# MoonLab-YH/AOD_MEH_HUA

Hardware: AMD Instinct MI355X
Metric: images/sec train+HUA-score, RetinaNet-R50 VOC 512^2 (higher is better)
Workload: dtype bf16x3

## Files before the change

### aod_meh_hua_amd/csrc/bottleneck_x3.hip

```cpp
#include "common.h"

namespace {

struct Bnx3Args {
  const bf16_t* x;
  const bf16_t* w1;
  const bf16_t* w2;
  const bf16_t* w3;
  const float* s1; const float* b1; const float* s2; const float* b2; const float* s3; const float* b3;
  const bf16_t* res;
  const bf16_t* wd; const float* sd; const float* bd;
  bf16_t* y;
  int B, H, W, CP, tiles_y, tiles_x;
  int st3;
};

constexpr int TH = 8, TW = 16, HW_ = 18, HPIX = (TH + 2) * HW_;
constexpr int M1 = 192;
constexpr int XBUF = M1 * 128;
constexpr int OFF_W1 = 2 * XBUF;
constexpr int OFF_T1 = 65536;
constexpr int T1SUB = M1 * 128, T2SUB = TH * TW * 128;
constexpr int OFF_VEC = OFF_T1 + 2 * T1SUB;
constexpr int NVEC = 1280;
constexpr int OFF_WD = OFF_VEC + NVEC * 4;
constexpr int LDS_BYTES = OFF_WD, LDS_BYTES_DS = OFF_WD + 32768;
constexpr int SLOT = 8192;
constexpr int W3SUB = 256 * 128;
static_assert(OFF_W1 + 2 * 8192 <= OFF_T1 && 8 * SLOT <= OFF_T1 && 2 * W3SUB <= OFF_T1 && 2 * T2SUB <= 2 * T1SUB && LDS_BYTES_DS <= 160 * 1024, "LDS map");

template <int N> __device__ __forceinline__ void wait_vm() { asm volatile("s_waitcnt vmcnt(%0)" ::"n"(N) : "memory"); }
#ifdef AOD_TILE_TIMING
__device__ unsigned long long* g_b64_stamps = nullptr;
#define BSTAMP(k) do { if (g_b64_stamps && threadIdx.x == 0) g_b64_stamps[(size_t)blockIdx.x * 8 + (k)] = wall_clock64(); } while (0)
#else
#define BSTAMP(k) do {} while (0)
#endif

__device__ __forceinline__ int xcd_remap(int bid, int nwg) {
  const int q = nwg >> 3, r = nwg & 7, xcd = bid & 7, j = bid >> 3;
  return (xcd < r ? xcd * (q + 1) : r * (q + 1) + (xcd - r) * q) + j;
}
__device__ __forceinline__ int swz(int row, int chunk) { return row * 128 + ((chunk ^ ((row >> 1) & 7)) << 4); }
__device__ __forceinline__ int wswz(int row, int chunk) { return row * 128 + ((chunk ^ ((row >> 1) & 7) ^ (((row >> 4) & 1) << 1)) << 4); }
__device__ __forceinline__ int wrow(int j, int lr) { return (j >> 1) * 32 + (lr >> 2) * 8 + (j & 1) * 4 + (lr & 3); }

__device__ __forceinline__ void split8(const float (&v)[8], bf16x8& h, bf16x8& l) {
#pragma unroll
  for (int j = 0; j < 8; ++j) { h[j] = (bf16_t)v[j]; l[j] = (bf16_t)(v[j] - (float)h[j]); }
}

template <bool DS>
__global__ __launch_bounds__(512) __attribute__((amdgpu_waves_per_eu(2, 2))) void bottleneck64x3_fwd_kernel(const Bnx3Args p) {
  extern __shared__ __attribute__((aligned(16))) char smem[];
  typedef unsigned u32x4_t __attribute__((ext_vector_type(4)));
  const int t = threadIdx.x, lane = t & 63;
  BSTAMP(0);
  const int uw = __builtin_amdgcn_readfirstlane(t >> 6);
  const int lr = lane & 15, lq = lane >> 4;
  const int ntile = p.tiles_y * p.tiles_x;
  const int wg = xcd_remap(blockIdx.x, p.B * ntile);
  const int b = wg / ntile, tt = wg - b * ntile;
  const int ty0 = (tt / p.tiles_x) * TH, tx0 = (tt % p.tiles_x) * TW;
  const long long img0 = (long long)b * p.H * p.W;
  const long long npix = (long long)p.B * p.H * p.W;
  const auto rsrc_x = __builtin_amdgcn_make_buffer_rsrc((void*)p.x, 0, (int)(npix * p.CP * 2), 0x00020000);
  const auto rsrc_w1 = __builtin_amdgcn_make_buffer_rsrc((void*)p.w1, 0, 64 * p.CP * 2, 0x00020000);
  const auto rsrc_w2 = __builtin_amdgcn_make_buffer_rsrc((void*)p.w2, 0, 64 * 9 * 128 * 2, 0x00020000);
  const auto rsrc_w3 = __builtin_amdgcn_make_buffer_rsrc((void*)p.w3, 0, 256 * 128 * 2, 0x00020000);
  const auto rsrc_res = __builtin_amdgcn_make_buffer_rsrc((void*)(DS ? p.x : p.res), 0, DS ? (int)(npix * p.CP * 2) : (int)(npix * 1024), 0x00020000);
  const auto rsrc_wd = __builtin_amdgcn_make_buffer_rsrc((void*)p.wd, 0, DS ? 256 * 128 * 2 : 0, 0x00020000);
  const auto rsrc_y = __builtin_amdgcn_make_buffer_rsrc((void*)p.y, 0, (int)(npix * 1024), 0x00020000);
  constexpr unsigned OOB = 0xf0000000u;
  const int drow = lane >> 3;
  const int kc = (lane & 7) ^ ((4 * (uw & 1) + (lane >> 4)) & 7);
  const int kcw = kc ^ (((uw >> 1) & 1) << 1);

  auto halo_pix = [&](int h, int& y, int& x) -> bool {
    const int hy = h / HW_, hx = h - hy * HW_;
    y = ty0 - 1 + hy; x = tx0 - 1 + hx;
    return h < HPIX && (unsigned)y < (unsigned)p.H && (unsigned)x < (unsigned)p.W;
  };
  float* const vec = reinterpret_cast<float*>(smem + OFF_VEC);
  {
    float v;
    if (t < 64) v = p.s1[t];
    else if (t < 128) v = p.b1[t - 64];
    else if (t < 192) v = p.s2[t - 128];
    else if (t < 256) v = p.b2[t - 192];
    else v = p.s3[t - 256];
    vec[t] = v;
    if (t < 256) vec[512 + t] = p.b3[t];
    if constexpr (DS) {
      if (t < 256) vec[768 + t] = p.sd[t]; else vec[768 + t] = p.bd[t - 256];
    }
  }
  const float* const vs1 = vec, * const vb1 = vec + 64, * const vs2 = vec + 128, * const vb2 = vec + 192, * const vs3 = vec + 256, * const vb3 = vec + 512;
  const float* const vsd = vec + 768, * const vbd = vec + 1024;
  const unsigned wdlane = (unsigned)((8 * uw + drow) * 256 + kcw * 16);
  auto issueD = [&](int half) {
#pragma unroll
    for (int g = 0; g < 2; ++g)
#pragma unroll
      for (int i = 0; i < 2; ++i)
        __builtin_amdgcn_raw_ptr_buffer_load_lds(rsrc_wd, (__attribute__((address_space(3))) void*)(smem + OFF_WD + g * 16384 + (uw + 8 * i) * 1024), 16,
                                                 wdlane + (unsigned)((half * 128 + i * 64) * 256) + (unsigned)g * 128u, 0, 0, 0);
  };
  if constexpr (DS) issueD(0);

  unsigned xoff[3];
#pragma unroll
  for (int i = 0; i < 3; ++i) {
    const int h = 8 * (uw + 8 * i) + drow;
    int y, x;
    xoff[i] = halo_pix(h, y, x) ? (unsigned)(((img0 + (long long)y * p.W + x) * p.CP + kc * 8) * 2) : OOB;
  }
  unsigned w1off = (unsigned)(((8 * uw + drow) * p.CP + kcw * 8) * 2);
  const int nk1 = p.CP >> 6;
  auto xstage = [&](int buf) -> char* { return smem + (buf < 2 ? buf * XBUF : OFF_T1); };
  auto wstage = [&](int buf) -> char* { return smem + (buf < 2 ? OFF_W1 + buf * 8192 : OFF_T1 + XBUF); };
  static_assert(OFF_T1 + XBUF + 8192 <= OFF_VEC, "third phase-1 stage inside the t1 region");
  auto issue1 = [&](int buf) {
    char* xs = xstage(buf);
#pragma unroll
    for (int i = 0; i < 3; ++i) {
      const unsigned off = xoff[i];
      __builtin_amdgcn_raw_ptr_buffer_load_lds(rsrc_x, (__attribute__((address_space(3))) void*)(xs + (uw + 8 * i) * 1024), 16, off, 0, 0, 0);
      xoff[i] += 128;
    }
    __builtin_amdgcn_raw_ptr_buffer_load_lds(rsrc_w1, (__attribute__((address_space(3))) void*)(wstage(buf) + uw * 1024), 16, w1off, 0, 0, 0);
    w1off += 128;
  };
  const bool two = uw < 4;
  f32x4 acc1[2][4];
#pragma unroll
  for (int i = 0; i < 2; ++i)
#pragma unroll
    for (int j = 0; j < 4; ++j) acc1[i][j] = (f32x4){0.f, 0.f, 0.f, 0.f};
  const int nst = p.st3 ? 3 : 2;
  issue1(0);
  if (nk1 > 1) issue1(1);
  if (nst > 2 && nk1 > 2) issue1(2);
  int buf = 0;
  for (int kt = 0; kt < nk1; ++kt) {
    const int young = min(nk1 - 1 - kt, nst - 1);
    if (young >= 2) wait_vm<8>(); else if (young == 1) wait_vm<4>(); else wait_vm<0>();
    __builtin_amdgcn_s_barrier();
    __builtin_amdgcn_sched_barrier(0);
    const char* xs = xstage(buf);
    const char* ws = wstage(buf);
    bf16x8 wh[4], wl[4];
#pragma unroll
    for (int j = 0; j < 4; ++j) {
      wh[j] = *reinterpret_cast<const bf16x8*>(ws + wswz(wrow(j, lr), lq));
      wl[j] = *reinterpret_cast<const bf16x8*>(ws + wswz(wrow(j, lr), 4 + lq));
    }
#pragma unroll
    for (int i = 0; i < 2; ++i) {
      if (i == 0 || two) {
        const int row = (uw + 8 * i) * 16 + lr;
        const bf16x8 xh = *reinterpret_cast<const bf16x8*>(xs + swz(row, lq)), xl = *reinterpret_cast<const bf16x8*>(xs + swz(row, 4 + lq));
#pragma unroll
        for (int j = 0; j < 4; ++j) {
          acc1[i][j] = __builtin_amdgcn_mfma_f32_16x16x32_bf16(wh[j], xh, acc1[i][j], 0, 0, 0);
          acc1[i][j] = __builtin_amdgcn_mfma_f32_16x16x32_bf16(wh[j], xl, acc1[i][j], 0, 0, 0);
          acc1[i][j] = __builtin_amdgcn_mfma_f32_16x16x32_bf16(wl[j], xh, acc1[i][j], 0, 0, 0);
        }
      }
    }
    __builtin_amdgcn_sched_barrier(0);
    asm volatile("s_waitcnt lgkmcnt(0)" ::: "memory");
    __builtin_amdgcn_s_barrier();
    if (kt + nst < nk1) issue1(buf);
    buf = buf == nst - 1 ? 0 : buf + 1;
  }
  BSTAMP(1);
  const unsigned w2lane = (unsigned)(((8 * uw + drow) * (9 * 128) + kcw * 8) * 2);
  auto issue2 = [&](int s) {
    __builtin_amdgcn_raw_ptr_buffer_load_lds(rsrc_w2, (__attribute__((address_space(3))) void*)(smem + (s & 7) * SLOT + uw * 1024), 16,
                                             w2lane + (unsigned)s * 128u, 0, 0, 0);
  };
#pragma unroll
  for (int s = 0; s < 8; ++s) issue2(s);
  {
    char* t1 = smem + OFF_T1;
#pragma unroll
    for (int i = 0; i < 2; ++i) {
      if (i == 0 || two) {
        const int h = (uw + 8 * i) * 16 + lr;
        int y, x;
        const bool ok = halo_pix(h, y, x);
#pragma unroll
        for (int jp = 0; jp < 2; ++jp) {
          const int c = jp * 32 + lq * 8;
          float v[8];
#pragma unroll
          for (int q = 0; q < 2; ++q) {
            const f32x4 sc = *reinterpret_cast<const f32x4*>(vs1 + c + 4 * q), sh = *reinterpret_cast<const f32x4*>(vb1 + c + 4 * q);
#pragma unroll
            for (int r = 0; r < 4; ++r) v[4 * q + r] = ok ? fmaxf(acc1[i][2 * jp + q][r] * sc[r] + sh[r], 0.f) : 0.f;
          }
          bf16x8 oh, ol;
          split8(v, oh, ol);
          *reinterpret_cast<bf16x8*>(t1 + jp * T1SUB + swz(h, lq)) = oh;
          *reinterpret_cast<bf16x8*>(t1 + jp * T1SUB + swz(h, 4 + lq)) = ol;
        }
      }
    }
  }

  BSTAMP(2);
  f32x4 acc2[4];
#pragma unroll
  for (int j = 0; j < 4; ++j) acc2[j] = (f32x4){0.f, 0.f, 0.f, 0.f};
  const unsigned w3lane = (unsigned)((8 * uw + drow) * 256 + kcw * 16);
  auto issue3 = [&](int g) {
#pragma unroll
    for (int i = 0; i < 4; ++i)
      __builtin_amdgcn_raw_ptr_buffer_load_lds(rsrc_w3, (__attribute__((address_space(3))) void*)(smem + g * W3SUB + (uw + 8 * i) * 1024), 16,
                                               w3lane + (unsigned)(i * 64 * 256) + (unsigned)g * 128u, 0, 0, 0);
  };
#pragma unroll
  for (int G = 0; G < 5; ++G) {
    const int nst = G < 4 ? 4 : 2;
    if (G == 0) wait_vm<4>();
    else if (G == 1) wait_vm<4>();
    else if (G == 2) wait_vm<4>();
    else if (G == 3) wait_vm<2>();
    else wait_vm<4>();
    asm volatile("s_waitcnt lgkmcnt(0)" ::: "memory");
    __builtin_amdgcn_s_barrier();
    __builtin_amdgcn_sched_barrier(0);
#pragma unroll
    for (int k = 0; k < nst; ++k) {
      const int s = 4 * G + k, tap = s >> 1, g = s & 1;
      const int r = tap / 3, q = tap - r * 3;
      const char* ws = smem + (s & 7) * SLOT;
      const char* t1 = smem + OFF_T1 + g * T1SUB;
      const int row = (uw + r) * HW_ + lr + q;
      const bf16x8 ah = *reinterpret_cast<const bf16x8*>(t1 + swz(row, lq)), al = *reinterpret_cast<const bf16x8*>(t1 + swz(row, 4 + lq));
#pragma unroll
      for (int j = 0; j < 4; ++j) {
        const bf16x8 fh = *reinterpret_cast<const bf16x8*>(ws + wswz(wrow(j, lr), lq)), fl = *reinterpret_cast<const bf16x8*>(ws + wswz(wrow(j, lr), 4 + lq));
        acc2[j] = __builtin_amdgcn_mfma_f32_16x16x32_bf16(fh, ah, acc2[j], 0, 0, 0);
        acc2[j] = __builtin_amdgcn_mfma_f32_16x16x32_bf16(fh, al, acc2[j], 0, 0, 0);
        acc2[j] = __builtin_amdgcn_mfma_f32_16x16x32_bf16(fl, ah, acc2[j], 0, 0, 0);
      }
    }
    __builtin_amdgcn_sched_barrier(0);
    asm volatile("s_waitcnt lgkmcnt(0)" ::: "memory");
    __builtin_amdgcn_s_barrier();
    if (G < 3) {
#pragma unroll
      for (int k = 0; k < 4; ++k) if (4 * (G + 2) + k < 18) issue2(4 * (G + 2) + k);
    } else if (G == 3) issue3(1);
    else issue3(0);
  }
  BSTAMP(3);
  {
    char* t2 = smem + OFF_T1;
    const int o_ = uw * 16 + lr;
#pragma unroll
    for (int jp = 0; jp < 2; ++jp) {
      const int c = jp * 32 + lq * 8;
      float v[8];
#pragma unroll
      for (int q = 0; q < 2; ++q) {
        const f32x4 sc = *reinterpret_cast<const f32x4*>(vs2 + c + 4 * q), sh = *reinterpret_cast<const f32x4*>(vb2 + c + 4 * q);
#pragma unroll
        for (int r = 0; r < 4; ++r) v[4 * q + r] = fmaxf(acc2[2 * jp + q][r] * sc[r] + sh[r], 0.f);
      }
      bf16x8 oh, ol;
      split8(v, oh, ol);
      *reinterpret_cast<bf16x8*>(t2 + jp * T2SUB + swz(o_, lq)) = oh;
      *reinterpret_cast<bf16x8*>(t2 + jp * T2SUB + swz(o_, 4 + lq)) = ol;
    }
  }
  const int oy = ty0 + uw, ox = tx0 + lr;
  const unsigned prow = (oy < p.H && ox < p.W) ? (unsigned)((img0 + (long long)oy * p.W + ox) * 1024) : OOB;
  u32x4_t rh[4], rl[4];
  auto load_res = [&](int half) {
#pragma unroll
    for (int jp = 0; jp < 4; ++jp) {
      const int c = half * 128 + jp * 32 + lq * 8;
      const unsigned col = (unsigned)((((c >> 5) << 6) + (c & 31)) * 2);
      rh[jp] = __builtin_amdgcn_raw_buffer_load_b128(rsrc_res, (int)(prow + col), 0, 0);
      rl[jp] = __builtin_amdgcn_raw_buffer_load_b128(rsrc_res, (int)(prow + col + 64u), 0, 0);
    }
  };
  u32x4_t xf[4];
  auto load_xf = [&]() {
    const unsigned xrow = (oy < p.H && ox < p.W) ? (unsigned)((img0 + (long long)oy * p.W + ox) * 256) : OOB;
#pragma unroll
    for (int q = 0; q < 4; ++q) xf[q] = __builtin_amdgcn_raw_buffer_load_b128(rsrc_res, (int)(xrow + (unsigned)(q * 64 + lq * 16)), 0, 0);
  };
  auto compute_res = [&](int half) {
    f32x4 accd[8];
#pragma unroll
    for (int j = 0; j < 8; ++j) accd[j] = (f32x4){0.f, 0.f, 0.f, 0.f};
#pragma unroll
    for (int g = 0; g < 2; ++g) {
      const char* ws = smem + OFF_WD + g * 16384;
      const bf16x8 ah = __builtin_bit_cast(bf16x8, xf[2 * g]), al = __builtin_bit_cast(bf16x8, xf[2 * g + 1]);
#pragma unroll
      for (int j = 0; j < 8; ++j) {
        const int fr = wrow(j, lr);
        const bf16x8 fh = *reinterpret_cast<const bf16x8*>(ws + wswz(fr, lq)), fl = *reinterpret_cast<const bf16x8*>(ws + wswz(fr, 4 + lq));
        accd[j] = __builtin_amdgcn_mfma_f32_16x16x32_bf16(fh, ah, accd[j], 0, 0, 0);
        accd[j] = __builtin_amdgcn_mfma_f32_16x16x32_bf16(fh, al, accd[j], 0, 0, 0);
        accd[j] = __builtin_amdgcn_mfma_f32_16x16x32_bf16(fl, ah, accd[j], 0, 0, 0);
      }
    }
#pragma unroll
    for (int jp = 0; jp < 4; ++jp) {
      const int c = half * 128 + jp * 32 + lq * 8;
      float v[8];
#pragma unroll
      for (int h2 = 0; h2 < 2; ++h2) {
        const f32x4 sc = *reinterpret_cast<const f32x4*>(vsd + c + 4 * h2), sh = *reinterpret_cast<const f32x4*>(vbd + c + 4 * h2);
#pragma unroll
        for (int r = 0; r < 4; ++r) v[4 * h2 + r] = accd[2 * jp + h2][r] * sc[r] + sh[r];
      }
      bf16x8 oh, ol;
      split8(v, oh, ol);
      rh[jp] = __builtin_bit_cast(u32x4_t, oh); rl[jp] = __builtin_bit_cast(u32x4_t, ol);
    }
  };
  wait_vm<0>();
  if constexpr (DS) load_xf(); else load_res(0);
  asm volatile("s_waitcnt lgkmcnt(0)" ::: "memory");
  __builtin_amdgcn_s_barrier();
  __builtin_amdgcn_sched_barrier(0);
  BSTAMP(4);

#pragma unroll
  for (int half = 0; half < 2; ++half) {
    if constexpr (DS) {
      if (half == 1) {
        wait_vm<12>();
        __builtin_amdgcn_s_barrier();
        __builtin_amdgcn_sched_barrier(0);
      }
      compute_res(half);
      if (half == 0) {
        __builtin_amdgcn_sched_barrier(0);
        asm volatile("s_waitcnt lgkmcnt(0)" ::: "memory");
        __builtin_amdgcn_s_barrier();
        issueD(1);
        __builtin_amdgcn_sched_barrier(0);
      }
    }
    f32x4 acc3[8];
#pragma unroll
    for (int j = 0; j < 8; ++j) acc3[j] = (f32x4){0.f, 0.f, 0.f, 0.f};
#pragma unroll
    for (int g = 0; g < 2; ++g) {
      const char* t2 = smem + OFF_T1 + g * T2SUB;
      const char* ws = smem + g * W3SUB;
      const int row = uw * 16 + lr;
      const bf16x8 ah = *reinterpret_cast<const bf16x8*>(t2 + swz(row, lq)), al = *reinterpret_cast<const bf16x8*>(t2 + swz(row, 4 + lq));
#pragma unroll
      for (int j = 0; j < 8; ++j) {
        const int fr = half * 128 + wrow(j, lr);
        const bf16x8 fh = *reinterpret_cast<const bf16x8*>(ws + wswz(fr, lq)), fl = *reinterpret_cast<const bf16x8*>(ws + wswz(fr, 4 + lq));
        acc3[j] = __builtin_amdgcn_mfma_f32_16x16x32_bf16(fh, ah, acc3[j], 0, 0, 0);
        acc3[j] = __builtin_amdgcn_mfma_f32_16x16x32_bf16(fh, al, acc3[j], 0, 0, 0);
        acc3[j] = __builtin_amdgcn_mfma_f32_16x16x32_bf16(fl, ah, acc3[j], 0, 0, 0);
      }
    }
#pragma unroll
    for (int jp = 0; jp < 4; ++jp) {
      const int c = half * 128 + jp * 32 + lq * 8;
      const u32x4_t qh = rh[jp], ql = rl[jp];
      float v[8];
#pragma unroll
      for (int h2 = 0; h2 < 2; ++h2) {
        const f32x4 sc = *reinterpret_cast<const f32x4*>(vs3 + c + 4 * h2), sh = *reinterpret_cast<const f32x4*>(vb3 + c + 4 * h2);
#pragma unroll
        for (int r = 0; r < 4; ++r) v[4 * h2 + r] = acc3[2 * jp + h2][r] * sc[r] + sh[r];
        v[4 * h2 + 0] += __uint_as_float(qh[2 * h2] << 16) + __uint_as_float(ql[2 * h2] << 16);
        v[4 * h2 + 1] += __uint_as_float(qh[2 * h2] & 0xffff0000u) + __uint_as_float(ql[2 * h2] & 0xffff0000u);
        v[4 * h2 + 2] += __uint_as_float(qh[2 * h2 + 1] << 16) + __uint_as_float(ql[2 * h2 + 1] << 16);
        v[4 * h2 + 3] += __uint_as_float(qh[2 * h2 + 1] & 0xffff0000u) + __uint_as_float(ql[2 * h2 + 1] & 0xffff0000u);
      }
#pragma unroll
      for (int r = 0; r < 8; ++r) v[r] = fmaxf(v[r], 0.f);
      bf16x8 oh, ol;
      split8(v, oh, ol);
      const unsigned col = (unsigned)((((c >> 5) << 6) + (c & 31)) * 2);
      __builtin_amdgcn_raw_buffer_store_b128(__builtin_bit_cast(u32x4_t, oh), rsrc_y, (int)(prow + col), 0, 0);
      __builtin_amdgcn_raw_buffer_store_b128(__builtin_bit_cast(u32x4_t, ol), rsrc_y, (int)(prow + col + 64u), 0, 0);
    }
    if (half == 0) { if constexpr (DS) { __builtin_amdgcn_sched_barrier(0); load_xf(); } else load_res(1); }
    BSTAMP(5 + half);
  }
#ifdef AOD_TILE_TIMING
  asm volatile("s_waitcnt vmcnt(0)" ::: "memory");
  BSTAMP(7);
#endif
}

}

#ifdef AOD_TILE_TIMING
extern "C" int aod_dbg_set_b64_stamps(void* buf) { return (int)hipMemcpyToSymbol(HIP_SYMBOL(g_b64_stamps), &buf, sizeof(buf)); }
#endif

static int launch_bnx3(const void* x, int Cin, int B, int H, int W, const void* w1, const float* s1, const float* b1, const void* w2,
                       const float* s2, const float* b2, const void* w3, const float* s3, const float* b3, const void* res, const void* wd,
                       const float* sd, const float* bd, void* y, aod_stream_t stream) {
  AOD_CHECK_ARG(x && w1 && w2 && w3 && s1 && b1 && s2 && b2 && s3 && b3 && y, "bottleneck64x3: null pointer");
  AOD_CHECK_ARG(Cin >= 32 && Cin % 32 == 0 && B >= 1 && H >= 1 && W >= 1, "bottleneck64x3: Cin %d must be a multiple of 32", Cin);
  AOD_CHECK_ARG((long long)B * H * W * (Cin > 256 ? Cin : 256) * 4 < 0xe0000000ll, "bottleneck64x3: operand larger than 3.5 GiB");
  Bnx3Args a;
  a.x = (const bf16_t*)x; a.w1 = (const bf16_t*)w1; a.w2 = (const bf16_t*)w2; a.w3 = (const bf16_t*)w3;
  a.s1 = s1; a.b1 = b1; a.s2 = s2; a.b2 = b2; a.s3 = s3; a.b3 = b3;
  a.res = (const bf16_t*)res; a.y = (bf16_t*)y;
  a.wd = (const bf16_t*)wd; a.sd = sd; a.bd = bd;
  a.B = B; a.H = H; a.W = W; a.CP = 2 * Cin;
  a.tiles_y = (H + TH - 1) / TH; a.tiles_x = (W + TW - 1) / TW;
  { const char* e = getenv("AOD_B64X3_ST3"); a.st3 = (e && e[0] == '0') ? 0 : 1; }
  static unsigned long long attr_done = 0;
  if (aod_first_on_device(&attr_done)) {
    (void)hipFuncSetAttribute(reinterpret_cast<const void*>(&bottleneck64x3_fwd_kernel<false>), hipFuncAttributeMaxDynamicSharedMemorySize, LDS_BYTES);
    (void)hipFuncSetAttribute(reinterpret_cast<const void*>(&bottleneck64x3_fwd_kernel<true>), hipFuncAttributeMaxDynamicSharedMemorySize, LDS_BYTES_DS);
  }
  if (wd) hipLaunchKernelGGL(bottleneck64x3_fwd_kernel<true>, dim3(B * a.tiles_y * a.tiles_x), dim3(512), LDS_BYTES_DS, (hipStream_t)stream, a);
  else hipLaunchKernelGGL(bottleneck64x3_fwd_kernel<false>, dim3(B * a.tiles_y * a.tiles_x), dim3(512), LDS_BYTES, (hipStream_t)stream, a);
  AOD_LAUNCH_CHECK();
  return 0;
}

extern "C" int aod_bottleneck64x3_fwd(const void* x, int Cin, int B, int H, int W, const void* w1, const float* s1, const float* b1, const void* w2,
                                      const float* s2, const float* b2, const void* w3, const float* s3, const float* b3, const void* res,
                                      void* y, aod_stream_t stream) {
  AOD_CHECK_ARG(res, "bottleneck64x3: null pointer");
  return launch_bnx3(x, Cin, B, H, W, w1, s1, b1, w2, s2, b2, w3, s3, b3, res, nullptr, nullptr, nullptr, y, stream);
}

extern "C" int aod_bottleneck64x3_ds_fwd(const void* x, int B, int H, int W, const void* w1, const float* s1, const float* b1, const void* w2,
                                         const float* s2, const float* b2, const void* w3, const float* s3, const float* b3, const void* wd,
                                         const float* sd, const float* bd, void* y, aod_stream_t stream) {
  AOD_CHECK_ARG(wd && sd && bd, "bottleneck64x3_ds: null pointer");
  return launch_bnx3(x, 64, B, H, W, w1, s1, b1, w2, s2, b2, w3, s3, b3, nullptr, wd, sd, bd, y, stream);
}
```

Baseline: 651.1.

## Process vertical runs of tiles per workgroup, reusing conv1 halo rows via ring buffer

Each workgroup now walks a vertical run of 8x16 tiles in one column strip instead of a single tile. The conv1 output is kept in a 10-row ring buffer, so later tiles only recompute the 8 new rows plus halo instead of all 10. This removes duplicated conv1 work on the halo and cuts per-tile launch overhead. The host picks the run length from the CU count to balance wave quantization against serialisation. The trade-off is less parallelism, a larger LDS footprint for the third stage in the non-downsample path, and more complex cross-tile synchronisation.

```diff
diff --git a/aod_meh_hua_amd/csrc/bottleneck_x3.hip b/aod_meh_hua_amd/csrc/bottleneck_x3.hip
--- a/aod_meh_hua_amd/csrc/bottleneck_x3.hip
+++ b/aod_meh_hua_amd/csrc/bottleneck_x3.hip
@@ -12,27 +12,31 @@
   const bf16_t* wd; const float* sd; const float* bd;
   bf16_t* y;
   int B, H, W, CP, tiles_y, tiles_x;
+  int run_len, runs_y;
   int st3;
 };
 
-constexpr int TH = 8, TW = 16, HW_ = 18, HPIX = (TH + 2) * HW_;
+constexpr int TH = 8, TW = 16, HW_ = 18, HROWS = TH + 2, HPIX = HROWS * HW_;
+constexpr int NPIX = TH * HW_;
 constexpr int M1 = 192;
 constexpr int XBUF = M1 * 128;
 constexpr int OFF_W1 = 2 * XBUF;
 constexpr int OFF_T1 = 65536;
-constexpr int T1SUB = M1 * 128, T2SUB = TH * TW * 128;
+constexpr int T1SUB = HPIX * 128;
 constexpr int OFF_VEC = OFF_T1 + 2 * T1SUB;
 constexpr int NVEC = 1280;
-constexpr int OFF_WD = OFF_VEC + NVEC * 4;
-constexpr int LDS_BYTES = OFF_WD, LDS_BYTES_DS = OFF_WD + 32768;
+constexpr int OFF_X3 = OFF_VEC + NVEC * 4;
+constexpr int OFF_WD = OFF_X3;
+constexpr int LDS_BYTES = OFF_X3 + XBUF + 8192, LDS_BYTES_DS = OFF_WD + 32768;
 constexpr int SLOT = 8192;
 constexpr int W3SUB = 256 * 128;
-static_assert(OFF_W1 + 2 * 8192 <= OFF_T1 && 8 * SLOT <= OFF_T1 && 2 * W3SUB <= OFF_T1 && 2 * T2SUB <= 2 * T1SUB && LDS_BYTES_DS <= 160 * 1024, "LDS map");
+static_assert(OFF_W1 + 2 * 8192 <= OFF_T1 && 8 * SLOT <= OFF_T1 && 2 * W3SUB <= OFF_T1 && (TH - 1) * HW_ + TW <= HPIX &&
+              LDS_BYTES <= 160 * 1024 && LDS_BYTES_DS <= 160 * 1024, "LDS map");
 
 template <int N> __device__ __forceinline__ void wait_vm() { asm volatile("s_waitcnt vmcnt(%0)" ::"n"(N) : "memory"); }
 #ifdef AOD_TILE_TIMING
 __device__ unsigned long long* g_b64_stamps = nullptr;
-#define BSTAMP(k) do { if (g_b64_stamps && threadIdx.x == 0) g_b64_stamps[(size_t)blockIdx.x * 8 + (k)] = wall_clock64(); } while (0)
+#define BSTAMP(k) do { if (g_b64_stamps && threadIdx.x == 0) g_b64_stamps[(size_t)tile_id * 8 + (k)] = wall_clock64(); } while (0)
 #else
 #define BSTAMP(k) do {} while (0)
 #endif
@@ -55,13 +59,14 @@
   extern __shared__ __attribute__((aligned(16))) char smem[];
   typedef unsigned u32x4_t __attribute__((ext_vector_type(4)));
   const int t = threadIdx.x, lane = t & 63;
-  BSTAMP(0);
   const int uw = __builtin_amdgcn_readfirstlane(t >> 6);
-  const int lr = lane & 15, lq = lane >> 4;
-  const int ntile = p.tiles_y * p.tiles_x;
-  const int wg = xcd_remap(blockIdx.x, p.B * ntile);
-  const int b = wg / ntile, tt = wg - b * ntile;
-  const int ty0 = (tt / p.tiles_x) * TH, tx0 = (tt % p.tiles_x) * TW;
+  int lr = lane & 15, lq = lane >> 4;
+  const int run = xcd_remap(blockIdx.x, (int)gridDim.x);
+  const int rpi = p.tiles_x * p.runs_y;
+  const int b = run / rpi, rr = run - b * rpi;
+  const int sx = rr / p.runs_y, ry = rr - sx * p.runs_y;
+  const int k0 = ry * p.run_len, k1 = min(k0 + p.run_len, p.tiles_y);
+  const int tx0 = sx * TW;
   const long long img0 = (long long)b * p.H * p.W;
   const long long npix = (long long)p.B * p.H * p.W;
   const auto rsrc_x = __builtin_amdgcn_make_buffer_rsrc((void*)p.x, 0, (int)(npix * p.CP * 2), 0x00020000);
@@ -76,10 +81,11 @@
   const int kc = (lane & 7) ^ ((4 * (uw & 1) + (lane >> 4)) & 7);
   const int kcw = kc ^ (((uw >> 1) & 1) << 1);
 
-  auto halo_pix = [&](int h, int& y, int& x) -> bool {
-    const int hy = h / HW_, hx = h - hy * HW_;
-    y = ty0 - 1 + hy; x = tx0 - 1 + hx;
-    return h < HPIX && (unsigned)y < (unsigned)p.H && (unsigned)x < (unsigned)p.W;
+  auto list_pix = [&](int h, bool first, int ty0, int& hr, int& hx, int& y, int& x) -> bool {
+    const int q = h / HW_;
+    hr = (first ? 0 : 2) + q; hx = h - q * HW_;
+    y = ty0 - 1 + hr; x = tx0 - 1 + hx;
+    return h < (first ? HPIX : NPIX) && (unsigned)y < (unsigned)p.H && (unsigned)x < (unsigned)p.W;
   };
   float* const vec = reinterpret_cast<float*>(smem + OFF_VEC);
   {
@@ -106,20 +112,21 @@
         __builtin_amdgcn_raw_ptr_buffer_load_lds(rsrc_wd, (__attribute__((address_space(3))) void*)(smem + OFF_WD + g * 16384 + (uw + 8 * i) * 1024), 16,
                                                  wdlane + (unsigned)((half * 128 + i * 64) * 256) + (unsigned)g * 128u, 0, 0, 0);
   };
-  if constexpr (DS) issueD(0);
-
-  unsigned xoff[3];
-#pragma unroll
-  for (int i = 0; i < 3; ++i) {
-    const int h = 8 * (uw + 8 * i) + drow;
-    int y, x;
-    xoff[i] = halo_pix(h, y, x) ? (unsigned)(((img0 + (long long)y * p.W + x) * p.CP + kc * 8) * 2) : OOB;
-  }
-  unsigned w1off = (unsigned)(((8 * uw + drow) * p.CP + kcw * 8) * 2);
+
   const int nk1 = p.CP >> 6;
-  auto xstage = [&](int buf) -> char* { return smem + (buf < 2 ? buf * XBUF : OFF_T1); };
-  auto wstage = [&](int buf) -> char* { return smem + (buf < 2 ? OFF_W1 + buf * 8192 : OFF_T1 + XBUF); };
-  static_assert(OFF_T1 + XBUF + 8192 <= OFF_VEC, "third phase-1 stage inside the t1 region");
+  const int nst = (!DS && p.st3) ? 3 : 2;
+  auto xstage = [&](int buf) -> char* { return DS ? smem + buf * XBUF : (buf == 0 ? smem + OFF_X3 : smem + (buf - 1) * XBUF); };
+  auto wstage = [&](int buf) -> char* { return DS ? smem + OFF_W1 + buf * 8192 : (buf == 0 ? smem + OFF_X3 + XBUF : smem + OFF_W1 + (buf - 1) * 8192); };
+  unsigned xoff[3], w1off;
+  auto setup1 = [&](int ty0, bool first) {
+#pragma unroll
+    for (int i = 0; i < 3; ++i) {
+      const int h = 8 * (uw + 8 * i) + drow;
+      int hr, hx, y, x;
+      xoff[i] = list_pix(h, first, ty0, hr, hx, y, x) ? (unsigned)(((img0 + (long long)y * p.W + x) * p.CP + kc * 8) * 2) : OOB;
+    }
+    w1off = (unsigned)(((8 * uw + drow) * p.CP + kcw * 8) * 2);
+  };
   auto issue1 = [&](int buf) {
     char* xs = xstage(buf);
 #pragma unroll
@@ -131,88 +138,11 @@
     __builtin_amdgcn_raw_ptr_buffer_load_lds(rsrc_w1, (__attribute__((address_space(3))) void*)(wstage(buf) + uw * 1024), 16, w1off, 0, 0, 0);
     w1off += 128;
   };
-  const bool two = uw < 4;
-  f32x4 acc1[2][4];
-#pragma unroll
-  for (int i = 0; i < 2; ++i)
-#pragma unroll
-    for (int j = 0; j < 4; ++j) acc1[i][j] = (f32x4){0.f, 0.f, 0.f, 0.f};
-  const int nst = p.st3 ? 3 : 2;
-  issue1(0);
-  if (nk1 > 1) issue1(1);
-  if (nst > 2 && nk1 > 2) issue1(2);
-  int buf = 0;
-  for (int kt = 0; kt < nk1; ++kt) {
-    const int young = min(nk1 - 1 - kt, nst - 1);
-    if (young >= 2) wait_vm<8>(); else if (young == 1) wait_vm<4>(); else wait_vm<0>();
-    __builtin_amdgcn_s_barrier();
-    __builtin_amdgcn_sched_barrier(0);
-    const char* xs = xstage(buf);
-    const char* ws = wstage(buf);
-    bf16x8 wh[4], wl[4];
-#pragma unroll
-    for (int j = 0; j < 4; ++j) {
-      wh[j] = *reinterpret_cast<const bf16x8*>(ws + wswz(wrow(j, lr), lq));
-      wl[j] = *reinterpret_cast<const bf16x8*>(ws + wswz(wrow(j, lr), 4 + lq));
-    }
-#pragma unroll
-    for (int i = 0; i < 2; ++i) {
-      if (i == 0 || two) {
-        const int row = (uw + 8 * i) * 16 + lr;
-        const bf16x8 xh = *reinterpret_cast<const bf16x8*>(xs + swz(row, lq)), xl = *reinterpret_cast<const bf16x8*>(xs + swz(row, 4 + lq));
-#pragma unroll
-        for (int j = 0; j < 4; ++j) {
-          acc1[i][j] = __builtin_amdgcn_mfma_f32_16x16x32_bf16(wh[j], xh, acc1[i][j], 0, 0, 0);
-          acc1[i][j] = __builtin_amdgcn_mfma_f32_16x16x32_bf16(wh[j], xl, acc1[i][j], 0, 0, 0);
-          acc1[i][j] = __builtin_amdgcn_mfma_f32_16x16x32_bf16(wl[j], xh, acc1[i][j], 0, 0, 0);
-        }
-      }
-    }
-    __builtin_amdgcn_sched_barrier(0);
-    asm volatile("s_waitcnt lgkmcnt(0)" ::: "memory");
-    __builtin_amdgcn_s_barrier();
-    if (kt + nst < nk1) issue1(buf);
-    buf = buf == nst - 1 ? 0 : buf + 1;
-  }
-  BSTAMP(1);
   const unsigned w2lane = (unsigned)(((8 * uw + drow) * (9 * 128) + kcw * 8) * 2);
   auto issue2 = [&](int s) {
     __builtin_amdgcn_raw_ptr_buffer_load_lds(rsrc_w2, (__attribute__((address_space(3))) void*)(smem + (s & 7) * SLOT + uw * 1024), 16,
                                              w2lane + (unsigned)s * 128u, 0, 0, 0);
   };
-#pragma unroll
-  for (int s = 0; s < 8; ++s) issue2(s);
-  {
-    char* t1 = smem + OFF_T1;
-#pragma unroll
-    for (int i = 0; i < 2; ++i) {
-      if (i == 0 || two) {
-        const int h = (uw + 8 * i) * 16 + lr;
-        int y, x;
-        const bool ok = halo_pix(h, y, x);
-#pragma unroll
-        for (int jp = 0; jp < 2; ++jp) {
-          const int c = jp * 32 + lq * 8;
-          float v[8];
-#pragma unroll
-          for (int q = 0; q < 2; ++q) {
-            const f32x4 sc = *reinterpret_cast<const f32x4*>(vs1 + c + 4 * q), sh = *reinterpret_cast<const f32x4*>(vb1 + c + 4 * q);
-#pragma unroll
-            for (int r = 0; r < 4; ++r) v[4 * q + r] = ok ? fmaxf(acc1[i][2 * jp + q][r] * sc[r] + sh[r], 0.f) : 0.f;
-          }
-          bf16x8 oh, ol;
-          split8(v, oh, ol);
-          *reinterpret_cast<bf16x8*>(t1 + jp * T1SUB + swz(h, lq)) = oh;
-          *reinterpret_cast<bf16x8*>(t1 + jp * T1SUB + swz(h, 4 + lq)) = ol;
-        }
-      }
-    }
-  }
-
-  BSTAMP(2);
-  f32x4 acc2[4];
-#pragma unroll
-  for (int j = 0; j < 4; ++j) acc2[j] = (f32x4){0.f, 0.f, 0.f, 0.f};
   const unsigned w3lane = (unsigned)((8 * uw + drow) * 256 + kcw * 16);
   auto issue3 = [&](int g) {
 #pragma unroll
@@ -220,184 +150,289 @@
       __builtin_amdgcn_raw_ptr_buffer_load_lds(rsrc_w3, (__attribute__((address_space(3))) void*)(smem + g * W3SUB + (uw + 8 * i) * 1024), 16,
                                                w3lane + (unsigned)(i * 64 * 256) + (unsigned)g * 128u, 0, 0, 0);
   };
-#pragma unroll
-  for (int G = 0; G < 5; ++G) {
-    const int nst = G < 4 ? 4 : 2;
-    if (G == 0) wait_vm<4>();
-    else if (G == 1) wait_vm<4>();
-    else if (G == 2) wait_vm<4>();
-    else if (G == 3) wait_vm<2>();
-    else wait_vm<4>();
+
+  bool pre = false;
+  for (int k = k0; k < k1; ++k) {
+    const bool first = k == k0;
+    const int ty0 = k * TH;
+#ifdef AOD_TILE_TIMING
+    const int tile_id = (b * p.tiles_y + k) * p.tiles_x + sx;
+#endif
+    const int sb = ((k - k0) * TH) % HROWS;
+    auto slot = [&](int hr) { const int s = sb + hr; return s >= HROWS ? s - HROWS : s; };
+    BSTAMP(0);
+    asm volatile("" : "+v"(lr), "+v"(lq));
+    if (!first) {
+      asm volatile("s_waitcnt lgkmcnt(0)" ::: "memory");
+      __builtin_amdgcn_s_barrier();
+      __builtin_amdgcn_sched_barrier(0);
+    }
+    if constexpr (DS) issueD(0);
+
+    if (!pre) { setup1(ty0, first); issue1(0); }
+    if (nk1 > 1) issue1(1);
+    if (nst > 2 && nk1 > 2) issue1(2);
+    const int nblk = first ? 12 : 9;
+    const bool two = uw + 8 < nblk;
+    f32x4 acc1[2][4];
+#pragma unroll
+    for (int i = 0; i < 2; ++i)
+#pragma unroll
+      for (int j = 0; j < 4; ++j) acc1[i][j] = (f32x4){0.f, 0.f, 0.f, 0.f};
+    int buf = 0;
+    for (int kt = 0; kt < nk1; ++kt) {
+      const int young = min(nk1 - 1 - kt, nst - 1);
+      if (young >= 2) wait_vm<8>(); else if (young == 1) wait_vm<4>(); else wait_vm<0>();
+      __builtin_amdgcn_s_barrier();
+      __builtin_amdgcn_sched_barrier(0);
+      const char* xs = xstage(buf);
+      const char* ws = wstage(buf);
+      bf16x8 wh[4], wl[4];
+#pragma unroll
+      for (int j = 0; j < 4; ++j) {
+        wh[j] = *reinterpret_cast<const bf16x8*>(ws + wswz(wrow(j, lr), lq));
+        wl[j] = *reinterpret_cast<const bf16x8*>(ws + wswz(wrow(j, lr), 4 + lq));
+      }
+#pragma unroll
+      for (int i = 0; i < 2; ++i) {
+        if (i == 0 || two) {
+          const int row = (uw + 8 * i) * 16 + lr;
+          const bf16x8 xh = *reinterpret_cast<const bf16x8*>(xs + swz(row, lq)), xl = *reinterpret_cast<const bf16x8*>(xs + swz(row, 4 + lq));
+#pragma unroll
+          for (int j = 0; j < 4; ++j) {
+            acc1[i][j] = __builtin_amdgcn_mfma_f32_16x16x32_bf16(wh[j], xh, acc1[i][j], 0, 0, 0);
+            acc1[i][j] = __builtin_amdgcn_mfma_f32_16x16x32_bf16(wh[j], xl, acc1[i][j], 0, 0, 0);
+            acc1[i][j] = __builtin_amdgcn_mfma_f32_16x16x32_bf16(wl[j], xh, acc1[i][j], 0, 0, 0);
+          }
+        }
+      }
+      __builtin_amdgcn_sched_barrier(0);
+      asm volatile("s_waitcnt lgkmcnt(0)" ::: "memory");
+      __builtin_amdgcn_s_barrier();
+      if (kt + nst < nk1) issue1(buf);
+      buf = buf == nst - 1 ? 0 : buf + 1;
+    }
+    BSTAMP(1);
+#pragma unroll
+    for (int s = 0; s < 8; ++s) issue2(s);
+    {
+      char* t1 = smem + OFF_T1;
+#pragma unroll
+      for (int i = 0; i < 2; ++i) {
+        if (i == 0 || two) {
+          const int h = (uw + 8 * i) * 16 + lr;
+          int hr, hx, y, x;
+          const bool ok = list_pix(h, first, ty0, hr, hx, y, x);
+          if (h < (first ? HPIX : NPIX)) {
+            const int e = slot(hr) * HW_ + hx;
+#pragma unroll
+            for (int jp = 0; jp < 2; ++jp) {
+              const int c = jp * 32 + lq * 8;
+              float v[8];
+#pragma unroll
+              for (int q = 0; q < 2; ++q) {
+                const f32x4 sc = *reinterpret_cast<const f32x4*>(vs1 + c + 4 * q), sh = *reinterpret_cast<const f32x4*>(vb1 + c + 4 * q);
+#pragma unroll
+                for (int r = 0; r < 4; ++r) v[4 * q + r] = ok ? fmaxf(acc1[i][2 * jp + q][r] * sc[r] + sh[r], 0.f) : 0.f;
+              }
+              bf16x8 oh, ol;
+              split8(v, oh, ol);
+              *reinterpret_cast<bf16x8*>(t1 + jp * T1SUB + swz(e, lq)) = oh;
+              *reinterpret_cast<bf16x8*>(t1 + jp * T1SUB + swz(e, 4 + lq)) = ol;
+            }
+          }
+        }
+      }
+    }
+
+    BSTAMP(2);
+    f32x4 acc2[4];
+#pragma unroll
+    for (int j = 0; j < 4; ++j) acc2[j] = (f32x4){0.f, 0.f, 0.f, 0.f};
+#pragma unroll
+    for (int G = 0; G < 5; ++G) {
+      const int ng = G < 4 ? 4 : 2;
+      if (G == 0) wait_vm<4>();
+      else if (G == 1) wait_vm<4>();
+      else if (G == 2) wait_vm<4>();
+      else if (G == 3) wait_vm<2>();
+      else wait_vm<4>();
+      asm volatile("s_waitcnt lgkmcnt(0)" ::: "memory");
+      __builtin_amdgcn_s_barrier();
+      __builtin_amdgcn_sched_barrier(0);
+#pragma unroll
+      for (int kk = 0; kk < ng; ++kk) {
+        const int s = 4 * G + kk, tap = s >> 1, g = s & 1;
+        const int r = tap / 3, q = tap - r * 3;
+        const char* ws = smem + (s & 7) * SLOT;
+        const char* t1 = smem + OFF_T1 + g * T1SUB;
+        const int row = slot(uw + r) * HW_ + lr + q;
+        const bf16x8 ah = *reinterpret_cast<const bf16x8*>(t1 + swz(row, lq)), al = *reinterpret_cast<const bf16x8*>(t1 + swz(row, 4 + lq));
+#pragma unroll
+        for (int j = 0; j < 4; ++j) {
+          const bf16x8 fh = *reinterpret_cast<const bf16x8*>(ws + wswz(wrow(j, lr), lq)), fl = *reinterpret_cast<const bf16x8*>(ws + wswz(wrow(j, lr), 4 + lq));
+          acc2[j] = __builtin_amdgcn_mfma_f32_16x16x32_bf16(fh, ah, acc2[j], 0, 0, 0);
+          acc2[j] = __builtin_amdgcn_mfma_f32_16x16x32_bf16(fh, al, acc2[j], 0, 0, 0);
+          acc2[j] = __builtin_amdgcn_mfma_f32_16x16x32_bf16(fl, ah, acc2[j], 0, 0, 0);
+        }
+      }
+      __builtin_amdgcn_sched_barrier(0);
+      asm volatile("s_waitcnt lgkmcnt(0)" ::: "memory");
+      __builtin_amdgcn_s_barrier();
+      if (G < 3) {
+#pragma unroll
+        for (int kk = 0; kk < 4; ++kk) if (4 * (G + 2) + kk < 18) issue2(4 * (G + 2) + kk);
+      } else if (G == 3) issue3(1);
+      else issue3(0);
+    }
+    BSTAMP(3);
+    const int t2row = slot(uw) * HW_ + lr;
+    {
+      char* t2 = smem + OFF_T1;
+#pragma unroll
+      for (int jp = 0; jp < 2; ++jp) {
+        const int c = jp * 32 + lq * 8;
+        float v[8];
+#pragma unroll
+        for (int q = 0; q < 2; ++q) {
+          const f32x4 sc = *reinterpret_cast<const f32x4*>(vs2 + c + 4 * q), sh = *reinterpret_cast<const f32x4*>(vb2 + c + 4 * q);
+#pragma unroll
+          for (int r = 0; r < 4; ++r) v[4 * q + r] = fmaxf(acc2[2 * jp + q][r] * sc[r] + sh[r], 0.f);
+        }
+        bf16x8 oh, ol;
+        split8(v, oh, ol);
+        *reinterpret_cast<bf16x8*>(t2 + jp * T1SUB + swz(t2row, lq)) = oh;
+        *reinterpret_cast<bf16x8*>(t2 + jp * T1SUB + swz(t2row, 4 + lq)) = ol;
+      }
+    }
+    const int oy = ty0 + uw, ox = tx0 + lr;
+    const unsigned prow = (oy < p.H && ox < p.W) ? (unsigned)((img0 + (long long)oy * p.W + ox) * 1024) : OOB;
+    u32x4_t rh[4], rl[4];
+    auto load_res = [&](int half) {
+#pragma unroll
+      for (int jp = 0; jp < 4; ++jp) {
+        const int c = half * 128 + jp * 32 + lq * 8;
+        const unsigned col = (unsigned)((((c >> 5) << 6) + (c & 31)) * 2);
+        rh[jp] = __builtin_amdgcn_raw_buffer_load_b128(rsrc_res, (int)(prow + col), 0, 0);
+        rl[jp] = __builtin_amdgcn_raw_buffer_load_b128(rsrc_res, (int)(prow + col + 64u), 0, 0);
+      }
+    };
+    u32x4_t xf[4];
+    auto load_xf = [&]() {
+      const unsigned xrow = (oy < p.H && ox < p.W) ? (unsigned)((img0 + (long long)oy * p.W + ox) * 256) : OOB;
+#pragma unroll
+      for (int q = 0; q < 4; ++q) xf[q] = __builtin_amdgcn_raw_buffer_load_b128(rsrc_res, (int)(xrow + (unsigned)(q * 64 + lq * 16)), 0, 0);
+    };
+    auto compute_res = [&](int half) {
+      f32x4 accd[8];
+#pragma unroll
+      for (int j = 0; j < 8; ++j) accd[j] = (f32x4){0.f, 0.f, 0.f, 0.f};
+#pragma unroll
+      for (int g = 0; g < 2; ++g) {
+        const char* ws = smem + OFF_WD + g * 16384;
+        const bf16x8 ah = __builtin_bit_cast(bf16x8, xf[2 * g]), al = __builtin_bit_cast(bf16x8, xf[2 * g + 1]);
+#pragma unroll
+        for (int j = 0; j < 8; ++j) {
+          const int fr = wrow(j, lr);
+          const bf16x8 fh = *reinterpret_cast<const bf16x8*>(ws + wswz(fr, lq)), fl = *reinterpret_cast<const bf16x8*>(ws + wswz(fr, 4 + lq));
+          accd[j] = __builtin_amdgcn_mfma_f32_16x16x32_bf16(fh, ah, accd[j], 0, 0, 0);
+          accd[j] = __builtin_amdgcn_mfma_f32_16x16x32_bf16(fh, al, accd[j], 0, 0, 0);
+          accd[j] = __builtin_amdgcn_mfma_f32_16x16x32_bf16(fl, ah, accd[j], 0, 0, 0);
+        }
+      }
+#pragma unroll
+      for (int jp = 0; jp < 4; ++jp) {
+        const int c = half * 128 + jp * 32 + lq * 8;
+        float v[8];
+#pragma unroll
+        for (int h2 = 0; h2 < 2; ++h2) {
+          const f32x4 sc = *reinterpret_cast<const f32x4*>(vsd + c + 4 * h2), sh = *reinterpret_cast<const f32x4*>(vbd + c + 4 * h2);
+#pragma unroll
+          for (int r = 0; r < 4; ++r) v[4 * h2 + r] = accd[2 * jp + h2][r] * sc[r] + sh[r];
+        }
+        bf16x8 oh, ol;
+        split8(v, oh, ol);
+        rh[jp] = __builtin_bit_cast(u32x4_t, oh); rl[jp] = __builtin_bit_cast(u32x4_t, ol);
+      }
+    };
+    wait_vm<0>();
+    if constexpr (DS) load_xf(); else load_res(0);
     asm volatile("s_waitcnt lgkmcnt(0)" ::: "memory");
     __builtin_amdgcn_s_barrier();
     __builtin_amdgcn_sched_barrier(0);
-#pragma unroll
-    for (int k = 0; k < nst; ++k) {
-      const int s = 4 * G + k, tap = s >> 1, g = s & 1;
-      const int r = tap / 3, q = tap - r * 3;
-      const char* ws = smem + (s & 7) * SLOT;
-      const char* t1 = smem + OFF_T1 + g * T1SUB;
-      const int row = (uw + r) * HW_ + lr + q;
-      const bf16x8 ah = *reinterpret_cast<const bf16x8*>(t1 + swz(row, lq)), al = *reinterpret_cast<const bf16x8*>(t1 + swz(row, 4 + lq));
-#pragma unroll
-      for (int j = 0; j < 4; ++j) {
-        const bf16x8 fh = *reinterpret_cast<const bf16x8*>(ws + wswz(wrow(j, lr), lq)), fl = *reinterpret_cast<const bf16x8*>(ws + wswz(wrow(j, lr), 4 + lq));
-        acc2[j] = __builtin_amdgcn_mfma_f32_16x16x32_bf16(fh, ah, acc2[j], 0, 0, 0);
-        acc2[j] = __builtin_amdgcn_mfma_f32_16x16x32_bf16(fh, al, acc2[j], 0, 0, 0);
-        acc2[j] = __builtin_amdgcn_mfma_f32_16x16x32_bf16(fl, ah, acc2[j], 0, 0, 0);
-      }
-    }
-    __builtin_amdgcn_sched_barrier(0);
-    asm volatile("s_waitcnt lgkmcnt(0)" ::: "memory");
-    __builtin_amdgcn_s_barrier();
-    if (G < 3) {
-#pragma unroll
-      for (int k = 0; k < 4; ++k) if (4 * (G + 2) + k < 18) issue2(4 * (G + 2) + k);
-    } else if (G == 3) issue3(1);
-    else issue3(0);
+    BSTAMP(4);
+    pre = !DS && k + 1 < k1;
+    if (pre) {
+      setup1(ty0 + TH, false);
+      issue1(0);
+      __builtin_amdgcn_sched_barrier(0);
+    }
+
+#pragma unroll
+    for (int half = 0; half < 2; ++half) {
+      if constexpr (DS) {
+        if (half == 1) {
+          wait_vm<12>();
+          __builtin_amdgcn_s_barrier();
+          __builtin_amdgcn_sched_barrier(0);
+        }
+        compute_res(half);
+        if (half == 0) {
+          __builtin_amdgcn_sched_barrier(0);
+          asm volatile("s_waitcnt lgkmcnt(0)" ::: "memory");
+          __builtin_amdgcn_s_barrier();
+          issueD(1);
+          __builtin_amdgcn_sched_barrier(0);
+        }
+      }
+      f32x4 acc3[8];
+#pragma unroll
+      for (int j = 0; j < 8; ++j) acc3[j] = (f32x4){0.f, 0.f, 0.f, 0.f};
+#pragma unroll
+      for (int g = 0; g < 2; ++g) {
+        const char* t2 = smem + OFF_T1 + g * T1SUB;
+        const char* ws = smem + g * W3SUB;
+        const bf16x8 ah = *reinterpret_cast<const bf16x8*>(t2 + swz(t2row, lq)), al = *reinterpret_cast<const bf16x8*>(t2 + swz(t2row, 4 + lq));
+#pragma unroll
+        for (int j = 0; j < 8; ++j) {
+          const int fr = half * 128 + wrow(j, lr);
+          const bf16x8 fh = *reinterpret_cast<const bf16x8*>(ws + wswz(fr, lq)), fl = *reinterpret_cast<const bf16x8*>(ws + wswz(fr, 4 + lq));
+          acc3[j] = __builtin_amdgcn_mfma_f32_16x16x32_bf16(fh, ah, acc3[j], 0, 0, 0);
+          acc3[j] = __builtin_amdgcn_mfma_f32_16x16x32_bf16(fh, al, acc3[j], 0, 0, 0);
+          acc3[j] = __builtin_amdgcn_mfma_f32_16x16x32_bf16(fl, ah, acc3[j], 0, 0, 0);
+        }
+      }
+#pragma unroll
+      for (int jp = 0; jp < 4; ++jp) {
+        const int c = half * 128 + jp * 32 + lq * 8;
+        const u32x4_t qh = rh[jp], ql = rl[jp];
+        float v[8];
+#pragma unroll
+        for (int h2 = 0; h2 < 2; ++h2) {
+          const f32x4 sc = *reinterpret_cast<const f32x4*>(vs3 + c + 4 * h2), sh = *reinterpret_cast<const f32x4*>(vb3 + c + 4 * h2);
+#pragma unroll
+          for (int r = 0; r < 4; ++r) v[4 * h2 + r] = acc3[2 * jp + h2][r] * sc[r] + sh[r];
+          v[4 * h2 + 0] += __uint_as_float(qh[2 * h2] << 16) + __uint_as_float(ql[2 * h2] << 16);
+          v[4 * h2 + 1] += __uint_as_float(qh[2 * h2] & 0xffff0000u) + __uint_as_float(ql[2 * h2] & 0xffff0000u);
+          v[4 * h2 + 2] += __uint_as_float(qh[2 * h2 + 1] << 16) + __uint_as_float(ql[2 * h2 + 1] << 16);
+          v[4 * h2 + 3] += __uint_as_float(qh[2 * h2 + 1] & 0xffff0000u) + __uint_as_float(ql[2 * h2 + 1] & 0xffff0000u);
+        }
+#pragma unroll
+        for (int r = 0; r < 8; ++r) v[r] = fmaxf(v[r], 0.f);
+        bf16x8 oh, ol;
+        split8(v, oh, ol);
+        const unsigned col = (unsigned)((((c >> 5) << 6) + (c & 31)) * 2);
+        __builtin_amdgcn_raw_buffer_store_b128(__builtin_bit_cast(u32x4_t, oh), rsrc_y, (int)(prow + col), 0, 0);
+        __builtin_amdgcn_raw_buffer_store_b128(__builtin_bit_cast(u32x4_t, ol), rsrc_y, (int)(prow + col + 64u), 0, 0);
+      }
+      if (half == 0) { if constexpr (DS) { __builtin_amdgcn_sched_barrier(0); load_xf(); } else load_res(1); }
+      BSTAMP(5 + half);
+    }
+#ifdef AOD_TILE_TIMING
+    asm volatile("s_waitcnt vmcnt(0)" ::: "memory");
+    BSTAMP(7);
+#endif
   }
-  BSTAMP(3);
-  {
-    char* t2 = smem + OFF_T1;
-    const int o_ = uw * 16 + lr;
-#pragma unroll
-    for (int jp = 0; jp < 2; ++jp) {
-      const int c = jp * 32 + lq * 8;
-      float v[8];
-#pragma unroll
-      for (int q = 0; q < 2; ++q) {
-        const f32x4 sc = *reinterpret_cast<const f32x4*>(vs2 + c + 4 * q), sh = *reinterpret_cast<const f32x4*>(vb2 + c + 4 * q);
-#pragma unroll
-        for (int r = 0; r < 4; ++r) v[4 * q + r] = fmaxf(acc2[2 * jp + q][r] * sc[r] + sh[r], 0.f);
-      }
-      bf16x8 oh, ol;
-      split8(v, oh, ol);
-      *reinterpret_cast<bf16x8*>(t2 + jp * T2SUB + swz(o_, lq)) = oh;
-      *reinterpret_cast<bf16x8*>(t2 + jp * T2SUB + swz(o_, 4 + lq)) = ol;
-    }
-  }
-  const int oy = ty0 + uw, ox = tx0 + lr;
-  const unsigned prow = (oy < p.H && ox < p.W) ? (unsigned)((img0 + (long long)oy * p.W + ox) * 1024) : OOB;
-  u32x4_t rh[4], rl[4];
-  auto load_res = [&](int half) {
-#pragma unroll
-    for (int jp = 0; jp < 4; ++jp) {
-      const int c = half * 128 + jp * 32 + lq * 8;
-      const unsigned col = (unsigned)((((c >> 5) << 6) + (c & 31)) * 2);
-      rh[jp] = __builtin_amdgcn_raw_buffer_load_b128(rsrc_res, (int)(prow + col), 0, 0);
-      rl[jp] = __builtin_amdgcn_raw_buffer_load_b128(rsrc_res, (int)(prow + col + 64u), 0, 0);
-    }
-  };
-  u32x4_t xf[4];
-  auto load_xf = [&]() {
-    const unsigned xrow = (oy < p.H && ox < p.W) ? (unsigned)((img0 + (long long)oy * p.W + ox) * 256) : OOB;
-#pragma unroll
-    for (int q = 0; q < 4; ++q) xf[q] = __builtin_amdgcn_raw_buffer_load_b128(rsrc_res, (int)(xrow + (unsigned)(q * 64 + lq * 16)), 0, 0);
-  };
-  auto compute_res = [&](int half) {
-    f32x4 accd[8];
-#pragma unroll
-    for (int j = 0; j < 8; ++j) accd[j] = (f32x4){0.f, 0.f, 0.f, 0.f};
-#pragma unroll
-    for (int g = 0; g < 2; ++g) {
-      const char* ws = smem + OFF_WD + g * 16384;
-      const bf16x8 ah = __builtin_bit_cast(bf16x8, xf[2 * g]), al = __builtin_bit_cast(bf16x8, xf[2 * g + 1]);
-#pragma unroll
-      for (int j = 0; j < 8; ++j) {
-        const int fr = wrow(j, lr);
-        const bf16x8 fh = *reinterpret_cast<const bf16x8*>(ws + wswz(fr, lq)), fl = *reinterpret_cast<const bf16x8*>(ws + wswz(fr, 4 + lq));
-        accd[j] = __builtin_amdgcn_mfma_f32_16x16x32_bf16(fh, ah, accd[j], 0, 0, 0);
-        accd[j] = __builtin_amdgcn_mfma_f32_16x16x32_bf16(fh, al, accd[j], 0, 0, 0);
-        accd[j] = __builtin_amdgcn_mfma_f32_16x16x32_bf16(fl, ah, accd[j], 0, 0, 0);
-      }
-    }
-#pragma unroll
-    for (int jp = 0; jp < 4; ++jp) {
-      const int c = half * 128 + jp * 32 + lq * 8;
-      float v[8];
-#pragma unroll
-      for (int h2 = 0; h2 < 2; ++h2) {
-        const f32x4 sc = *reinterpret_cast<const f32x4*>(vsd + c + 4 * h2), sh = *reinterpret_cast<const f32x4*>(vbd + c + 4 * h2);
-#pragma unroll
-        for (int r = 0; r < 4; ++r) v[4 * h2 + r] = accd[2 * jp + h2][r] * sc[r] + sh[r];
-      }
-      bf16x8 oh, ol;
-      split8(v, oh, ol);
-      rh[jp] = __builtin_bit_cast(u32x4_t, oh); rl[jp] = __builtin_bit_cast(u32x4_t, ol);
-    }
-  };
-  wait_vm<0>();
-  if constexpr (DS) load_xf(); else load_res(0);
-  asm volatile("s_waitcnt lgkmcnt(0)" ::: "memory");
-  __builtin_amdgcn_s_barrier();
-  __builtin_amdgcn_sched_barrier(0);
-  BSTAMP(4);
-
-#pragma unroll
-  for (int half = 0; half < 2; ++half) {
-    if constexpr (DS) {
-      if (half == 1) {
-        wait_vm<12>();
-        __builtin_amdgcn_s_barrier();
-        __builtin_amdgcn_sched_barrier(0);
-      }
-      compute_res(half);
-      if (half == 0) {
-        __builtin_amdgcn_sched_barrier(0);
-        asm volatile("s_waitcnt lgkmcnt(0)" ::: "memory");
-        __builtin_amdgcn_s_barrier();
-        issueD(1);
-        __builtin_amdgcn_sched_barrier(0);
-      }
-    }
-    f32x4 acc3[8];
-#pragma unroll
-    for (int j = 0; j < 8; ++j) acc3[j] = (f32x4){0.f, 0.f, 0.f, 0.f};
-#pragma unroll
-    for (int g = 0; g < 2; ++g) {
-      const char* t2 = smem + OFF_T1 + g * T2SUB;
-      const char* ws = smem + g * W3SUB;
-      const int row = uw * 16 + lr;
-      const bf16x8 ah = *reinterpret_cast<const bf16x8*>(t2 + swz(row, lq)), al = *reinterpret_cast<const bf16x8*>(t2 + swz(row, 4 + lq));
-#pragma unroll
-      for (int j = 0; j < 8; ++j) {
-        const int fr = half * 128 + wrow(j, lr);
-        const bf16x8 fh = *reinterpret_cast<const bf16x8*>(ws + wswz(fr, lq)), fl = *reinterpret_cast<const bf16x8*>(ws + wswz(fr, 4 + lq));
-        acc3[j] = __builtin_amdgcn_mfma_f32_16x16x32_bf16(fh, ah, acc3[j], 0, 0, 0);
-        acc3[j] = __builtin_amdgcn_mfma_f32_16x16x32_bf16(fh, al, acc3[j], 0, 0, 0);
-        acc3[j] = __builtin_amdgcn_mfma_f32_16x16x32_bf16(fl, ah, acc3[j], 0, 0, 0);
-      }
-    }
-#pragma unroll
-    for (int jp = 0; jp < 4; ++jp) {
-      const int c = half * 128 + jp * 32 + lq * 8;
-      const u32x4_t qh = rh[jp], ql = rl[jp];
-      float v[8];
-#pragma unroll
-      for (int h2 = 0; h2 < 2; ++h2) {
-        const f32x4 sc = *reinterpret_cast<const f32x4*>(vs3 + c + 4 * h2), sh = *reinterpret_cast<const f32x4*>(vb3 + c + 4 * h2);
-#pragma unroll
-        for (int r = 0; r < 4; ++r) v[4 * h2 + r] = acc3[2 * jp + h2][r] * sc[r] + sh[r];
-        v[4 * h2 + 0] += __uint_as_float(qh[2 * h2] << 16) + __uint_as_float(ql[2 * h2] << 16);
-        v[4 * h2 + 1] += __uint_as_float(qh[2 * h2] & 0xffff0000u) + __uint_as_float(ql[2 * h2] & 0xffff0000u);
-        v[4 * h2 + 2] += __uint_as_float(qh[2 * h2 + 1] << 16) + __uint_as_float(ql[2 * h2 + 1] << 16);
-        v[4 * h2 + 3] += __uint_as_float(qh[2 * h2 + 1] & 0xffff0000u) + __uint_as_float(ql[2 * h2 + 1] & 0xffff0000u);
-      }
-#pragma unroll
-      for (int r = 0; r < 8; ++r) v[r] = fmaxf(v[r], 0.f);
-      bf16x8 oh, ol;
-      split8(v, oh, ol);
-      const unsigned col = (unsigned)((((c >> 5) << 6) + (c & 31)) * 2);
-      __builtin_amdgcn_raw_buffer_store_b128(__builtin_bit_cast(u32x4_t, oh), rsrc_y, (int)(prow + col), 0, 0);
-      __builtin_amdgcn_raw_buffer_store_b128(__builtin_bit_cast(u32x4_t, ol), rsrc_y, (int)(prow + col + 64u), 0, 0);
-    }
-    if (half == 0) { if constexpr (DS) { __builtin_amdgcn_sched_barrier(0); load_xf(); } else load_res(1); }
-    BSTAMP(5 + half);
-  }
-#ifdef AOD_TILE_TIMING
-  asm volatile("s_waitcnt vmcnt(0)" ::: "memory");
-  BSTAMP(7);
-#endif
 }
 
 }
@@ -405,6 +440,18 @@
 #ifdef AOD_TILE_TIMING
 extern "C" int aod_dbg_set_b64_stamps(void* buf) { return (int)hipMemcpyToSymbol(HIP_SYMBOL(g_b64_stamps), &buf, sizeof(buf)); }
 #endif
+
+static int bnx3_cus() {
+  static int cus[64];
+  int dev = 0;
+  if (hipGetDevice(&dev) != hipSuccess || dev < 0 || dev > 63) dev = 0;
+  if (!cus[dev]) {
+    int n = 0;
+    if (hipDeviceGetAttribute(&n, hipDeviceAttributeMultiprocessorCount, dev) != hipSuccess || n <= 0) n = 256;
+    cus[dev] = n;
+  }
+  return cus[dev];
+}
 
 static int launch_bnx3(const void* x, int Cin, int B, int H, int W, const void* w1, const float* s1, const float* b1, const void* w2,
                        const float* s2, const float* b2, const void* w3, const float* s3, const float* b3, const void* res, const void* wd,
@@ -419,14 +466,25 @@
   a.wd = (const bf16_t*)wd; a.sd = sd; a.bd = bd;
   a.B = B; a.H = H; a.W = W; a.CP = 2 * Cin;
   a.tiles_y = (H + TH - 1) / TH; a.tiles_x = (W + TW - 1) / TW;
+  const int ncu = bnx3_cus();
+  const long long strips = (long long)B * a.tiles_x;
+  double best = 1e300;
+  for (int L = 1; L <= a.tiles_y; ++L) {
+    const long long runs = strips * ((a.tiles_y + L - 1) / L);
+    const double c = (double)((runs + ncu - 1) / ncu) * (L + 0.25);
+    if (c < best) { best = c; a.run_len = L; }
+  }
+  a.runs_y = (a.tiles_y + a.run_len - 1) / a.run_len;
+  const long long nwg = strips * a.runs_y;
+  AOD_CHECK_ARG(nwg < 0x7fffffffll, "bottleneck64x3: too many workgroups");
   { const char* e = getenv("AOD_B64X3_ST3"); a.st3 = (e && e[0] == '0') ? 0 : 1; }
   static unsigned long long attr_done = 0;
   if (aod_first_on_device(&attr_done)) {
     (void)hipFuncSetAttribute(reinterpret_cast<const void*>(&bottleneck64x3_fwd_kernel<false>), hipFuncAttributeMaxDynamicSharedMemorySize, LDS_BYTES);
     (void)hipFuncSetAttribute(reinterpret_cast<const void*>(&bottleneck64x3_fwd_kernel<true>), hipFuncAttributeMaxDynamicSharedMemorySize, LDS_BYTES_DS);
   }
-  if (wd) hipLaunchKernelGGL(bottleneck64x3_fwd_kernel<true>, dim3(B * a.tiles_y * a.tiles_x), dim3(512), LDS_BYTES_DS, (hipStream_t)stream, a);
-  else hipLaunchKernelGGL(bottleneck64x3_fwd_kernel<false>, dim3(B * a.tiles_y * a.tiles_x), dim3(512), LDS_BYTES, (hipStream_t)stream, a);
+  if (wd) hipLaunchKernelGGL(bottleneck64x3_fwd_kernel<true>, dim3((unsigned)nwg), dim3(512), LDS_BYTES_DS, (hipStream_t)stream, a);
+  else hipLaunchKernelGGL(bottleneck64x3_fwd_kernel<false>, dim3((unsigned)nwg), dim3(512), LDS_BYTES, (hipStream_t)stream, a);
   AOD_LAUNCH_CHECK();
   return 0;
 }
```

Result: no change. 653.8, median of 6 (+0.4%).
